# voichek/kmersGWAS

Hardware: AMD Instinct MI355X
Metric: k-mers x permutations scored/sec (higher is better)
Workload: dtype fp4 x fp6/fp4 block-scaled filter + f32/f64 exact re-score

## Files before the change

kmersgwas_amd/csrc/aux_kernels.hip:

```cpp
#include "score_common.h"
#include "synth.h"

namespace kgwas {

static hipError_t ensure_dyn_lds(const void* fn, size_t bytes) {
    if (bytes > 64 * 1024) return hipFuncSetAttribute(fn, hipFuncAttributeMaxDynamicSharedMemorySize, (int)bytes);
    return hipSuccess;
}

__global__ void __launch_bounds__(256) squeeze_kernel(const uint64_t* file_rows, uint64_t file_stride_w,
                                                      uint64_t n_rows, const uint32_t* colmap, uint32_t W_m,
                                                      uint32_t W_f, uint32_t* out) {
    extern __shared__ uint32_t lds_u32[];
    const uint32_t in_dw = 2u * W_f, in_ld = in_dw + 1u;
    const uint32_t out_dw = 2u * W_m, out_ld = out_dw + 1u;
    uint32_t* lin = lds_u32;
    uint32_t* lout = lds_u32 + 64u * in_ld;
    const uint64_t row0 = (uint64_t)blockIdx.x * 64u;
    const uint32_t* fr = reinterpret_cast<const uint32_t*>(file_rows);

    for (uint32_t e = threadIdx.x; e < 64u * in_dw; e += 256u) {
        const uint32_t rr = e / in_dw, dw = e - rr * in_dw;
        const uint64_t gr = row0 + rr;
        lin[rr * in_ld + dw] = (gr < n_rows) ? fr[gr * file_stride_w * 2u + 2u + dw] : 0u;
// ... 245 lines not shown
                                                         unsigned long long* __restrict__ h_tested, const double* __restrict__ thr, uint32_t n_thr,
                                                         double* __restrict__ h_thr) {
    for (uint32_t i = threadIdx.x; i < n_meta; i += 256u) h_meta[i] = meta[i];
    for (uint32_t i = threadIdx.x; i < n_tested; i += 256u) h_tested[i] = tested[i];
    for (uint32_t i = threadIdx.x; i < n_thr; i += 256u) h_thr[i] = thr[i];
}

hipError_t launch_chunk_tail(const uint32_t* meta, uint32_t n_meta, uint32_t* h_meta, const unsigned long long* tested, uint32_t n_tested,
                             unsigned long long* h_tested, const double* thr, uint32_t n_thr, double* h_thr, hipStream_t st) {
    launch_last(chunk_tail_kernel, dim3(1), dim3(256), 0, st, meta, n_meta, h_meta, tested, n_tested, h_tested, thr, n_thr, h_thr);
    return hipGetLastError();
}

__global__ void __launch_bounds__(256) thr_tail_kernel(const uint32_t* hist, const uint32_t* hist_base, uint32_t bins, const uint64_t* topn,
                                                       const double* thr_host, double* thr, const uint32_t* __restrict__ meta, uint32_t n_meta,
                                                       uint32_t* __restrict__ h_meta, const unsigned long long* __restrict__ tested, uint32_t n_tested,
                                                       unsigned long long* __restrict__ h_tested, double* __restrict__ h_thr) {
    thr_update_block(hist, hist_base, bins, topn, thr_host, thr, blockIdx.x);
    if (h_thr && threadIdx.x == 0) h_thr[blockIdx.x] = thr[blockIdx.x];
    if (blockIdx.x == 0) {
        for (uint32_t i = threadIdx.x; i < n_meta; i += 256u) h_meta[i] = meta[i];
        for (uint32_t i = threadIdx.x; i < n_tested; i += 256u) h_tested[i] = tested[i];
    }
}

hipError_t launch_thr_tail(const uint32_t* hist, const uint32_t* hist_base, uint32_t bins, const uint64_t* topn, const double* thr_host, double* thr,
                           uint32_t n_pheno, const uint32_t* meta, uint32_t n_meta, uint32_t* h_meta, const unsigned long long* tested,
                           uint32_t n_tested, unsigned long long* h_tested, double* h_thr, hipStream_t st) {
    if (n_pheno == 0 || bins % 256u) return hipErrorInvalidValue;
    launch_last(thr_tail_kernel, dim3(n_pheno), dim3(256), 0, st, hist, hist_base, bins, topn, thr_host, thr, meta, n_meta, h_meta, tested,
                n_tested, h_tested, h_thr);
    return hipGetLastError();
}

hipError_t launch_records_to_host(const double* sc, const uint64_t* km, const uint32_t* rw, uint32_t n, double* h_sc, uint64_t* h_km, uint32_t* h_rw,
                                  hipStream_t st) {
    if (!n) return hipSuccess;
    static const uint32_t max_blocks = (uint64_t)exp_int("KGWAS_RECORD_BLOCKS", 64u);
    const uint32_t blocks = std::min<uint32_t>((n + 255u) / 256u, std::max(1u, max_blocks));
    hipLaunchKernelGGL(records_to_host_kernel, dim3(blocks), dim3(256), 0, st, reinterpret_cast<const unsigned long long*>(sc),
                       reinterpret_cast<const unsigned long long*>(km), rw, n, reinterpret_cast<unsigned long long*>(h_sc),
                       reinterpret_cast<unsigned long long*>(h_km), h_rw);
    return hipGetLastError();
}

hipError_t launch_thr_update(const uint32_t* hist, const uint32_t* hist_base, uint32_t bins, const uint64_t* topn,
// ... 47 lines not shown
```

kmersgwas_amd/csrc/kernels.h:

```cpp
#pragma once
#include <hip/hip_runtime.h>
#include <stdint.h>

#include "env.h"
#include "launch.h"

namespace kgwas {

struct Cand {
    uint64_t kmer;
    double score;
    uint64_t row;
};

struct RowSrc {
    const uint32_t* base;
    uint64_t stride_dw;
    uint32_t off_dw;
    uint32_t avail_dw;
};

constexpr uint32_t TESTED_SHARDS = 256;

struct ScoreArgs {
// ... 20 lines not shown
    unsigned long long* tested;
    uint32_t* hist;
    const uint32_t* hist_base;
    uint32_t hist_bins;
    double* so_score;
    uint64_t* so_kmer;
    uint32_t* so_row;
};

constexpr int HIST_SHIFT = 44;
constexpr uint32_t HIST_BINS = 16384;

hipError_t launch_copy_to_host(const void* src, void* dst_dev, size_t bytes, hipStream_t st);
hipError_t launch_chunk_tail(const uint32_t* meta, uint32_t n_meta, uint32_t* h_meta, const unsigned long long* tested, uint32_t n_tested,
                             unsigned long long* h_tested, const double* thr, uint32_t n_thr, double* h_thr, hipStream_t st);
hipError_t launch_thr_tail(const uint32_t* hist, const uint32_t* hist_base, uint32_t bins, const uint64_t* topn, const double* thr_host, double* thr,
                           uint32_t n_pheno, const uint32_t* meta, uint32_t n_meta, uint32_t* h_meta, const unsigned long long* tested,
                           uint32_t n_tested, unsigned long long* h_tested, double* h_thr, hipStream_t st);
hipError_t launch_records_to_host(const double* sc, const uint64_t* km, const uint32_t* rw, uint32_t n, double* h_sc, uint64_t* h_km, uint32_t* h_rw,
                                  hipStream_t st);
hipError_t launch_thr_update(const uint32_t* hist, const uint32_t* hist_base, uint32_t bins, const uint64_t* topn,
                             const double* thr_host, double* thr, uint32_t n_pheno, hipStream_t st);

hipError_t launch_dense_select(const double* dense, const uint32_t* n1, uint32_t n_rows, uint32_t n_pheno, uint32_t S, uint32_t min_count,
                               const uint64_t* topn, double* thr_a, double* thr_b, double* thr_host_copy, uint32_t* info, hipStream_t st);

hipError_t launch_score_valu(const ScoreArgs& a, hipStream_t st);
hipError_t launch_score_mfma(const ScoreArgs& a, uint32_t rows_per_block, uint32_t nb_full, hipStream_t st);
size_t mfma_lds_bytes(uint32_t W_m);

struct CoarseCol {
    double kalpha;
    float iu;
// ... 73 lines not shown
    uint32_t S, n_pheno, min_count;
    uint32_t n_kgroups;
    const uint8_t* Bn;
    const NarrowCol* cols;
    const double* thr;
    unsigned long long* bitmap;
    uint64_t words_per_col;
    unsigned long long* tested;
    uint32_t row_off;
    uint32_t* seg_cnt;
    uint32_t n_segs;
    uint64_t slack_rows;
    uint32_t pack1;
};
hipError_t launch_bitmap_keys(unsigned long long* bitmap, uint64_t words_per_col, uint64_t n_rows, uint32_t n_pheno, uint32_t* blk_scratch,
                              unsigned long long* blk_mask, uint32_t* keys_sorted, uint32_t key_cap, uint32_t row_bits, uint32_t* surv_off,
                              uint32_t* surv_cnt, uint32_t* key_count, uint32_t* tile_pref, bool nibble_transposed, hipStream_t st);
hipError_t launch_narrow_keys(const unsigned long long* bitmap, uint64_t words_per_col, uint64_t n_rows, uint32_t n_pheno, const uint32_t* seg_cnt,
                              uint32_t* keys_sorted, uint32_t key_cap, uint32_t row_bits, uint32_t* surv_off, uint32_t* surv_cnt,
                              uint32_t* key_count, uint32_t* tile_pref, uint32_t* meta, const unsigned long long* tested_shards, hipStream_t st);
size_t narrow_lds_bytes(uint32_t n_kgroups);
hipError_t launch_narrow(const NarrowArgs& a, uint32_t rows_per_block, hipStream_t st);

hipError_t launch_pattern_hash(const RowSrc& src, const uint32_t* dmask, uint64_t n_rows, uint32_t S, uint32_t W_m,
                               uint32_t min_count, uint64_t* out, unsigned long long* out_count, hipStream_t st);
hipError_t count_distinct_u64(uint64_t* keys, uint64_t n, uint64_t* result, hipStream_t st);

hipError_t launch_bed_rowinfo(const uint32_t* sq, uint64_t n_rows, uint32_t W_m, uint32_t* n1_out, uint64_t* hash_out,
                              hipStream_t st);
hipError_t launch_bed_bytes(const uint32_t* sq, uint64_t n_rows, uint32_t W_m, uint32_t bytes_per_row, uint8_t* out,
                            hipStream_t st);

// ... 95 lines not shown
```

kmersgwas_amd/csrc/launch.h:

```cpp
#pragma once
#include <hip/hip_runtime.h>

#include <tuple>
#include <utility>

extern "C" hipError_t hipExtLaunchKernel(const void* function_address, dim3 numBlocks, dim3 dimBlocks, void** args, size_t sharedMemBytes,
                                         hipStream_t stream, hipEvent_t startEvent, hipEvent_t stopEvent, int flags);

namespace kgwas {

extern thread_local hipEvent_t g_bound_stop;

template <class... KA, size_t... I>
inline hipError_t launch_bound_impl(void (*kernel)(KA...), dim3 grid, dim3 block, size_t lds, hipStream_t st, hipEvent_t stop, std::tuple<KA...>& vals,
                                    std::index_sequence<I...>) {
    void* ptrs[] = {const_cast<void*>(static_cast<const void*>(&std::get<I>(vals)))..., nullptr};
    return hipExtLaunchKernel(reinterpret_cast<const void*>(kernel), grid, block, ptrs, lds, st, nullptr, stop, 0);
}

template <class... KA, class... A>
inline void launch_last(void (*kernel)(KA...), dim3 grid, dim3 block, size_t lds, hipStream_t st, A&&... args) {
    static_assert(sizeof...(KA) == sizeof...(A), "one argument per kernel parameter");
    const hipEvent_t stop = g_bound_stop;
    g_bound_stop = nullptr;
    if (!stop) {
        hipLaunchKernelGGL(kernel, grid, block, lds, st, static_cast<KA>(args)...);
        return;
    }
    std::tuple<KA...> vals(static_cast<KA>(args)...);
    (void)launch_bound_impl(kernel, grid, block, lds, st, stop, vals, std::index_sequence_for<KA...>{});
}

template <class F>
inline hipError_t bind_stop(hipEvent_t ev, hipStream_t st, F&& launcher) {
    g_bound_stop = ev;
    const hipError_t e = launcher();
    if (g_bound_stop) {
        g_bound_stop = nullptr;
        if (e == hipSuccess) return hipEventRecord(ev, st);
    }
    return e;
}

}
```

kmersgwas_amd/csrc/scan_create.cpp:

```cpp
#include "scan_internal.h"
#include <chrono>

struct CreateTrace {
    const bool on = opt_set("KGWAS_TRACE");
    const std::chrono::steady_clock::time_point t0 = std::chrono::steady_clock::now();
    void operator()(const char* what) const {
        if (on)
            fprintf(stderr, "[kgwas] scan_create +%.1f ms: %s\n", std::chrono::duration<double, std::milli>(std::chrono::steady_clock::now() - t0).count(), what);
    }
};

static std::unique_ptr<kgwas_scan> new_session(const kgwas_scan_params* p, ScanShape& sh) {
    if (p->struct_size != sizeof(kgwas_scan_params)) throw Error(KGWAS_ERR_ARG, "kgwas_scan_params: size mismatch");
    if (!p->col || !p->Y || !p->topn || p->n_acc == 0 || p->n_pheno == 0 || p->n_acc_file == 0)
        throw Error(KGWAS_ERR_ARG, "kgwas_scan_create: empty problem");
    if (p->n_acc > p->n_acc_file) throw Error(KGWAS_ERR_ARG, "more phenotyped accessions than table columns");
    if (p->n_acc_file >= (1ull << 31)) throw Error(KGWAS_ERR_ARG, "too many accessions");
    require_heap_emulation();
    check_device(p->device);
    KGWAS_HIP(hipSetDevice(p->device));
    std::unique_ptr<kgwas_scan> s(new kgwas_scan);
    s->device = p->device;
    s->S_f = p->n_acc_file;
    s->S = p->n_acc;
// ... 142 lines not shown
            if (pl.use_mx) s->st.coarse_mx = 1;
            s->st.coarse_mx_s1_fp6 = fs.s1_fp6;
            s->st.coarse_mx_steps = fs.n_steps;
        }
        M.ready = true;
    }
}

static void alloc_filter_buffers(kgwas_scan* s) {
    const uint64_t P = s->n_pheno;
    s->key_slots = (uint32_t)std::min<uint64_t>((uint64_t)s->cap * P, 0x7FFFFFFFull);
    s->d_surv_sorted.alloc(s->key_slots);
    s->bitmap_words = (s->chunk_max + 63) / 64;
    s->d_bitmap.alloc(P * s->bitmap_words);
    s->d_bm_blocks.alloc(P * ((s->bitmap_words + 1023) / 1024 + 1) + 4);
    if (!s->narrow) s->d_bm_mask.alloc(P * ((s->bitmap_words + 1023) / 1024) * 4 + 4);
    s->bitmap_clean = false;
    s->d_surv_cnt.alloc(P);
    s->d_surv_off.alloc(P);
    s->d_key_count.alloc(2);
    s->d_tile_pref.alloc(P + 1);
    s->d_tile_cnt.alloc((size_t)s->key_slots / 256 + P + 2);
    s->d_tmp_score.alloc(s->key_slots);
    int least = 0, greatest = 0;
    KGWAS_HIP(hipDeviceGetStreamPriorityRange(&least, &greatest));
    const bool hi = !(exp_int("KGWAS_COPY_PRIO", 1) == 0);
    KGWAS_HIP(hipStreamCreateWithPriority(&s->copy_stream, hipStreamNonBlocking, hi ? greatest : least));
    s->row_key_bits = 1;
    while (s->row_key_bits < 32 && (1ull << s->row_key_bits) < s->chunk_max) s->row_key_bits++;
}

// ... 172 lines not shown
```

kmersgwas_amd/csrc/scan_gpu.cpp:

```cpp
#include "scan_internal.h"

namespace kgwas {


void fill_args(kgwas_scan* s, ScoreArgs& a, const uint64_t* d_rows, uint64_t n_rows, uint64_t first_row,
               bool squeezed) {
    memset(&a, 0, sizeof(a));
    if (squeezed) {
        a.src.base = s->d_sq.p;
        a.src.stride_dw = 2 * s->W_m;
        a.src.off_dw = 0;
        a.src.avail_dw = (uint32_t)(2 * s->W_m);
    } else {
        a.src.base = reinterpret_cast<const uint32_t*>(d_rows);
        a.src.stride_dw = 2 * (1 + s->W_f);
        a.src.off_dw = 2;
        a.src.avail_dw = (uint32_t)(2 * s->W_f);
    }
    a.dmask = s->d_dmask.p;
    a.file_rows = d_rows;
    a.file_stride_w = 1 + s->W_f;
    a.n_rows = n_rows;
    a.first_row = first_row;
    a.S = (uint32_t)s->S;
// ... 302 lines not shown
            tu.hist = s->d_hist.p;
            tu.hist_base = s->d_hist_base.p;
            tu.bins = HIST_BINS;
            tu.topn = s->d_topn.p;
            tu.thr_host = s->d_thr_host.p;
            tu.thr = s->d_thr.p;
        }
        const bool zero_bitmap = use_coarse && (s->narrow || !s->bitmap_clean);
        const uint64_t zero_words = !zero_bitmap ? 0 : (s->narrow ? s->n_pheno * n_words : s->d_bitmap.n);
        const auto prep = [&] {
            return launch_chunk_prep(sl.d_cnt.p, (uint32_t)s->n_pheno, sl.d_tested.p, use_coarse ? s->d_key_count.p : nullptr,
                                     zero_bitmap ? s->d_bitmap.p : nullptr, zero_words,
                                     (use_coarse && s->narrow) ? s->d_bm_blocks.p : nullptr, (use_coarse && s->narrow) ? (uint32_t)s->n_pheno * n_segs : 0u,
                                     tu, s->stream);
        };
        if (s->direct) KGWAS_HIP(bind_stop(sl.ev_k0, s->stream, prep));
        else KGWAS_HIP(prep());
    }
    sl.used_coarse = use_coarse;
    if (use_coarse) {
        CoarseArgs c;
        memset(&c, 0, sizeof(c));
        c.src = a.src;
        c.n_rows = n_rows;
        c.S = a.S;
        c.n_pheno = a.n_pheno;
        c.min_count = a.min_count;
        c.n_kgroups = s->n_kgroups;
        const int cm = s->narrow ? 0 : pick_coarse_mode(s);
        if (s->dbg_keep_surv) dbg_log_thresholds(s, a.thr, n_rows, first_row, s->narrow ? 2u : (uint32_t)cm);
        const kgwas_scan::CoarseMode& M = s->cmode[cm];
        sl.coarse_mode = cm;
// ... 60 lines not shown
                    x.tested = c.tested;
                    x.eg_max = c.eg_max;
                    x.rall_max = c.rall_max;
                    x.rmax_max = c.rmax_max;
                    const auto filt = [&] {
                        return Pt.stream ? launch_mxs(x, Pt.T, Pt.ng, Pt.stream - 1u, rpb, s->stream) : launch_mx(x, Pt.T, rpb, s->stream);
                    };
                    if (last_part) KGWAS_HIP(bind_stop(sl.ev_mid, s->stream, filt));
                    else KGWAS_HIP(filt());
                } else {
                    const auto filt = [&] { return launch_coarse(c, Pt.T, rpb, s->stream); };
                    if (last_part) KGWAS_HIP(bind_stop(sl.ev_mid, s->stream, filt));
                    else KGWAS_HIP(filt());
                }
            }
            if (!M.n_parts) KGWAS_HIP(hipEventRecord(sl.ev_mid, s->stream));
        }
        a.tested = nullptr;
        a.so_score = sl.d_so_score.p;
        a.so_kmer = sl.d_so_kmer.p;
        a.so_row = sl.d_so_row.p;
        if (s->narrow) {
            KGWAS_HIP(launch_narrow_keys(s->d_bitmap.p, n_words, n_rows, (uint32_t)s->n_pheno, s->d_bm_blocks.p, s->d_surv_sorted.p, s->key_slots,
                                         s->row_key_bits, s->d_surv_off.p, s->d_surv_cnt.p, s->d_key_count.p, s->d_tile_pref.p, sl.d_meta.p, sl.d_tested.p, s->stream));
            if (s->dbg_keep_surv) dbg_log_survivors(s);
            KGWAS_HIP(bind_stop(sl.ev_k1, s->stream, [&] { return launch_rescore_direct(a, s->d_surv_sorted.p, s->d_surv_off.p, s->d_surv_cnt.p, s->row_key_bits, s->d_tile_pref.p, s->stream); }));
        } else {
        KGWAS_HIP(launch_bitmap_keys(s->d_bitmap.p, n_words, n_rows, (uint32_t)s->n_pheno, s->d_bm_blocks.p, s->d_bm_mask.p, s->d_surv_sorted.p, s->key_slots,
                                     s->row_key_bits, s->d_surv_off.p, s->d_surv_cnt.p, s->d_key_count.p, s->d_tile_pref.p, !s->narrow, s->stream));
        s->bitmap_clean = true;
        if (s->dbg_keep_surv) dbg_log_survivors(s);
        a.so_score = sl.d_so_score.p;
        a.so_kmer = sl.d_so_kmer.p;
        a.so_row = sl.d_so_row.p;
        KGWAS_HIP(bind_stop(sl.ev_k1, s->stream, [&] {
            return launch_rescore(a, s->d_surv_sorted.p, s->d_surv_off.p, s->d_surv_cnt.p, s->row_key_bits, s->d_tile_pref.p,
                                  s->d_tile_cnt.p, s->d_tmp_score.p, s->d_key_count.p, sl.d_meta.p, s->stream);
        }));
        }
        s->st.score_launches++;
    } else {
        if (s->direct) KGWAS_HIP(hipEventRecord(sl.ev_k0, s->stream));
        launch_score(s, a);
        KGWAS_HIP(hipEventRecord(sl.ev_k1, s->stream));
// ... 2 lines not shown
    static const bool tail_kernel = !(exp_int("KGWAS_TAIL_KERNEL", 1) == 0);
    const bool one_launch = use_coarse && tail_kernel && sl.h_meta_dev;
    const bool thr_and_tail = one_launch && s->hist_ready && !fused_tail;
    if (s->hist_ready && !fused_tail && !thr_and_tail)
        KGWAS_HIP(launch_thr_update(s->d_hist.p, s->d_hist_base.p, HIST_BINS, s->d_topn.p, s->d_thr_host.p, s->d_thr.p,
                                    (uint32_t)s->n_pheno, s->stream));
    if (!fused_tail && !one_launch)
        KGWAS_HIP(hipMemcpyAsync(sl.h_tested.p, sl.d_tested.p, TESTED_SHARDS * sizeof(unsigned long long), hipMemcpyDeviceToHost,
                                 s->stream));
    sl.tested_in_meta = fused_tail;
    if (thr_and_tail) {
        const bool thr_too = s->lazy_any.load(std::memory_order_relaxed);
        KGWAS_HIP(bind_stop(sl.ev_counts, s->stream, [&] {
            return launch_thr_tail(s->d_hist.p, s->d_hist_base.p, HIST_BINS, s->d_topn.p, s->d_thr_host.p, s->d_thr.p, (uint32_t)s->n_pheno, sl.d_meta.p,
                                   (uint32_t)(2 * s->n_pheno + 4), sl.h_meta_dev, sl.d_tested.p, (uint32_t)TESTED_SHARDS, sl.h_tested_dev,
                                   thr_too ? sl.h_thr_dev : nullptr, s->stream);
        }));
    } else if (one_launch) {
        const bool thr_too = s->lazy_any.load(std::memory_order_relaxed);
        KGWAS_HIP(bind_stop(sl.ev_counts, s->stream, [&] {
            return launch_chunk_tail(sl.d_meta.p, (uint32_t)(2 * s->n_pheno + 4), sl.h_meta_dev, sl.d_tested.p, fused_tail ? 0u : (uint32_t)TESTED_SHARDS,
                                     sl.h_tested_dev, s->d_thr.p, thr_too ? (uint32_t)s->n_pheno : 0u, sl.h_thr_dev, s->stream);
        }));
    } else if (use_coarse) {
        KGWAS_HIP(hipMemcpyAsync(sl.h_meta.p, sl.d_meta.p, (2 * s->n_pheno + 4) * sizeof(uint32_t), hipMemcpyDeviceToHost, s->stream));
        if (s->lazy_any.load(std::memory_order_relaxed))
            KGWAS_HIP(hipMemcpyAsync(sl.h_thr.p, s->d_thr.p, s->n_pheno * sizeof(double), hipMemcpyDeviceToHost, s->stream));
        KGWAS_HIP(hipEventRecord(sl.ev_counts, s->stream));
    } else {
        KGWAS_HIP(hipMemcpyAsync(sl.h_cnt.p, sl.d_cnt.p, s->n_pheno * sizeof(uint32_t), hipMemcpyDeviceToHost, s->stream));
        KGWAS_HIP(hipEventRecord(sl.ev_done, s->stream));
    }
// ... 19 lines not shown
        s->st.coarse_mode_rows[sl.coarse_mode] += sl.n_rows;
    }
    if (!s->direct) {
        float mq = 0;
        KGWAS_HIP(hipEventElapsedTime(&mq, sl.ev_sq0, sl.ev_k0));
        s->st.squeeze_kernel_ms += mq;
    }
    bool over = false;
    if (sl.used_coarse) {
        over = sl.h_meta.p[2 * s->n_pheno + 1] > s->key_slots;
    } else {
        for (uint64_t j = 0; j < s->n_pheno && !over; j++) over = sl.h_cnt.p[j] > s->cap;
    }
    if (s->trace) {
        uint64_t tot = 0, mx = 0;
        for (uint64_t q = 0; q < s->n_pheno; q++) {
            const uint64_t v = sl.used_coarse ? sl.h_meta.p[q] : sl.h_cnt.p[q];
            tot += v;
            mx = std::max<uint64_t>(mx, v);
        }
        fprintf(stderr, "[kgwas] chunk rows=%llu first=%llu kernel=%.3fms records %llu (max per column %llu)%s%s\n",
                (unsigned long long)sl.n_rows, (unsigned long long)sl.first_row, ms, (unsigned long long)tot,
                (unsigned long long)mx, sl.used_coarse ? (" survivors " + std::to_string(sl.h_meta.p[2 * s->n_pheno + 1])).c_str() : "",
                over ? " OVERFLOW" : "");
    }
    if (over) return false;
    if (sl.tested_in_meta)
        s->st.rows_tested += (uint64_t)sl.h_meta.p[2 * s->n_pheno + 2] | ((uint64_t)sl.h_meta.p[2 * s->n_pheno + 3] << 32);
    else
        for (uint32_t i = 0; i < TESTED_SHARDS; i++) s->st.rows_tested += sl.h_tested.p[i];
    return true;
}

uint64_t next_sparse_chunk(const kgwas_scan* s) {
    const double m = (double)std::max<uint64_t>(s->rows_submitted, 1);
    static const double fill_env = exp_num("KGWAS_FILL", 0.0);
    const double fill = fill_env > 0.0 ? fill_env : (s->narrow ? (s->lazy_any.load(std::memory_order_relaxed) ? 0.15 : 0.05) : 0.4);
// ... 98 lines not shown
```

kmersgwas_amd/csrc/scan_host.cpp:

```cpp
#include "scan_internal.h"
#include <sched.h>

namespace kgwas {

thread_local hipEvent_t g_bound_stop = nullptr;


std::vector<int> parse_cpulist(const char* path) {
    std::vector<int> out;
    FILE* f = fopen(path, "r");
    if (!f) return out;
    char buf[4096];
    if (fgets(buf, sizeof(buf), f)) {
        for (char* tok = strtok(buf, ",\n"); tok; tok = strtok(nullptr, ",\n")) {
            int a = 0, b = 0;
            const int k = sscanf(tok, "%d-%d", &a, &b);
            if (k == 1) b = a;
            if (k >= 1)
                for (int c = a; c <= b; c++) out.push_back(c);
        }
    }
    fclose(f);
    return out;
}
// ... 197 lines not shown
```

kmersgwas_amd/csrc/scan_internal.h:

```cpp
#pragma once
#include <algorithm>
#include <atomic>
#include <chrono>
#include <cmath>
#include <condition_variable>
#include <deque>
#include <limits>
#include <cstdio>
#include <cstdlib>
#include <cstring>
#include <functional>
#include <memory>
#include <mutex>
#include <string>
#include <thread>
#include <vector>

#include <dirent.h>
#include <immintrin.h>
#include <pthread.h>
#include <sched.h>
#include <sys/mman.h>

#include "common.h"
// ... 303 lines not shown
    double* so_score = nullptr;
    uint64_t* so_kmer = nullptr;
    uint32_t* so_row = nullptr;
    size_t ring_end = 0;
    DevBuf<double> d_so_score;
    DevBuf<uint64_t> d_so_kmer;
    DevBuf<uint32_t> d_so_row;
    DevBuf<uint32_t> d_meta;
    PinBuf<uint32_t> h_meta;
    uint32_t* h_meta_dev = nullptr;
    double* h_thr_dev = nullptr;
    unsigned long long* h_tested_dev = nullptr;
    PinBuf<double> h_thr;
    bool tie_check = false;
    bool tested_in_meta = false;
    hipEvent_t ev_counts = nullptr;
    DevBuf<unsigned long long> d_tested;
    PinBuf<unsigned long long> h_tested;
    hipEvent_t ev_sq0 = nullptr, ev_k0 = nullptr, ev_k1 = nullptr, ev_done = nullptr, ev_mid = nullptr;
    bool used_coarse = false;
    int coarse_mode = 0;
    double cand_est = 0;
    const uint64_t* rows = nullptr;
    uint64_t first_row = 0, n_rows = 0;
    bool squeezed = false, busy = false;
};

}

using namespace kgwas;
// ... 53 lines not shown
    PinBuf<uint32_t> h_sel_info;
    bool sel_valid = false;
    double infl_obs[2] = {4.0, 1.1};
    double mode_k = 0;
    std::chrono::steady_clock::time_point t_feed0;
    double t_ms() const { return std::chrono::duration<double, std::milli>(std::chrono::steady_clock::now() - t_feed0).count(); }
    uint64_t sum_topn = 0;
    bool narrow = false;
    bool narrow_pack1 = false;
    DevBuf<uint8_t> d_Bn;
    DevBuf<NarrowCol> d_ncols;
    DevBuf<unsigned long long> d_bitmap;
    uint64_t bitmap_words = 0;
    DevBuf<uint32_t> d_bm_blocks;
    DevBuf<unsigned long long> d_bm_mask;
    bool bitmap_clean = false;
    uint64_t slack_rows = 0;
    DevBuf<uint32_t> d_surv_sorted, d_surv_cnt, d_surv_off, d_key_count;
    DevBuf<uint32_t> d_tile_pref, d_tile_cnt;
    DevBuf<double> d_tmp_score;
    uint32_t key_slots = 0;
    uint32_t row_key_bits = 32;
    bool count_patterns = false;
    DevBuf<uint64_t> d_pat;
    DevBuf<unsigned long long> d_pat_cnt;
    uint64_t pat_upper = 0;
    Slot slot[MAX_SLOTS];
    PinBuf<uint8_t> ring;
    uint8_t* ring_dev = nullptr;
    bool streamed_feed = false;
// ... 208 lines not shown
```

kmersgwas_amd/csrc/score_narrow.hip:

```cpp
#include <stdlib.h>

#include <algorithm>

#include "score_common.h"

#ifndef KGWAS_NARROW_ABLATE
#define KGWAS_NARROW_ABLATE 0
#endif

namespace kgwas {

typedef int nv8i __attribute__((ext_vector_type(8)));
typedef float nv4f __attribute__((ext_vector_type(4)));

namespace {
constexpr int NRT = 4;
}

__device__ __forceinline__ void narrow_group(const uint32_t (&piece)[NRT][4], const uint4* sg, nv4f (&acc)[NRT]) {
#pragma unroll
    for (int j = 0; j < 4; j++) {
        uint4 s0, s1;
        if (KGWAS_NARROW_ABLATE & 16) {
            s0 = make_uint4(j, 1, 2, 3);
// ... 337 lines not shown
#undef NARROW_EACH
#undef NARROW_LOAD
#undef NARROW_PUT
    __syncthreads();
    narrow_flush_counts(a, L);
    if (a.tested) {
        uint32_t v = tested_local;
#pragma unroll
        for (int dd = 1; dd < 64; dd <<= 1) v += __shfl_xor(v, dd);
        if (lane == 0u && v) atomicAdd(&a.tested[blockIdx.x % TESTED_SHARDS], (unsigned long long)v);
    }
}

constexpr uint32_t BM_WORDS = 1024;

__global__ void __launch_bounds__(256) bitmap_count_kernel(const unsigned long long* bm, uint64_t words_per_col, uint32_t n_words,
                                                           uint32_t n_blocks, uint32_t* blk_cnt, unsigned long long* blk_mask) {
    __shared__ uint32_t part[4];
    const uint32_t p = blockIdx.y, b = blockIdx.x;
    const unsigned long long* w = bm + (uint64_t)p * words_per_col;
    uint32_t c = 0;
#pragma unroll
    for (int i = 0; i < 4; i++) {
        const uint32_t x = b * BM_WORDS + threadIdx.x * 4u + i;
        if (x < n_words) c += __popcll(w[x]);
    }
    const unsigned long long m = __ballot(c != 0u);
    if ((threadIdx.x & 63u) == 0u) blk_mask[((uint64_t)p * n_blocks + b) * 4u + (threadIdx.x >> 6)] = m;
#pragma unroll
    for (int d = 1; d < 64; d <<= 1) c += __shfl_xor(c, d);
    if ((threadIdx.x & 63u) == 0u) part[threadIdx.x >> 6] = c;
    __syncthreads();
    if (threadIdx.x == 0) blk_cnt[p * n_blocks + b] = part[0] + part[1] + part[2] + part[3];
}

__global__ void __launch_bounds__(256) bitmap_scan_kernel(uint32_t* blk_cnt, uint32_t n_blocks, uint32_t* col_total) {
    __shared__ uint32_t part[256];
    __shared__ uint32_t carry;
    const uint32_t p = blockIdx.x;
    if (threadIdx.x == 0) carry = 0;
    __syncthreads();
    for (uint32_t b0 = 0; b0 < n_blocks; b0 += 256u) {
        const uint32_t b = b0 + threadIdx.x;
        const uint32_t v = b < n_blocks ? blk_cnt[p * n_blocks + b] : 0u;
        part[threadIdx.x] = v;
        __syncthreads();
        for (uint32_t d = 1; d < 256u; d <<= 1) {
            const uint32_t x = threadIdx.x >= d ? part[threadIdx.x - d] : 0u;
            __syncthreads();
            part[threadIdx.x] += x;
            __syncthreads();
        }
        if (b < n_blocks) blk_cnt[p * n_blocks + b] = carry + part[threadIdx.x] - v;
        __syncthreads();
        if (threadIdx.x == 255u) carry += part[255];
        __syncthreads();
    }
    if (threadIdx.x == 0) col_total[p] = carry;
}

__device__ __forceinline__ void bitmap_bases_block(const uint32_t* col_total, uint32_t n_pheno, uint32_t key_cap, uint32_t* surv_off,
                                                   uint32_t* surv_cnt, uint32_t* key_count, uint32_t* tile_pref) {
    __shared__ uint32_t part[256];
    __shared__ uint32_t carry;
    if (threadIdx.x == 0) carry = 0;
    __syncthreads();
    for (uint32_t p0 = 0; p0 < n_pheno; p0 += 256u) {
        const uint32_t p = p0 + threadIdx.x;
        const uint32_t v = p < n_pheno ? col_total[p] : 0u;
        part[threadIdx.x] = v;
        __syncthreads();
        for (uint32_t d = 1; d < 256u; d <<= 1) {
            const uint32_t x = threadIdx.x >= d ? part[threadIdx.x - d] : 0u;
// ... 25 lines not shown
            const uint32_t x = threadIdx.x >= d ? part[threadIdx.x - d] : 0u;
            __syncthreads();
            part[threadIdx.x] += x;
            __syncthreads();
        }
        if (p < n_pheno) tile_pref[p] = carry + part[threadIdx.x] - v;
        __syncthreads();
        if (threadIdx.x == 255u) carry += part[255];
        __syncthreads();
    }
    if (threadIdx.x == 0) tile_pref[n_pheno] = carry;
    __syncthreads();
}

__global__ void __launch_bounds__(256) bitmap_scatter_kernel(unsigned long long* bm, uint64_t words_per_col, uint32_t n_words,
                                                             uint32_t n_blocks, const uint32_t* blk_off, const uint32_t* col_total,
                                                             const unsigned long long* blk_mask, uint32_t n_pheno, uint32_t* surv_off,
                                                             uint32_t* surv_cnt, uint32_t* key_count, uint32_t* tile_pref, uint32_t* keys,
                                                             uint32_t key_cap, uint32_t row_bits, bool nibble_transposed) {
    __shared__ uint32_t part[4];
    __shared__ uint32_t basep[4];
    const uint32_t p = blockIdx.y, b = blockIdx.x;
    if (p == 0u && b == 0u) bitmap_bases_block(col_total, n_pheno, key_cap, surv_off, surv_cnt, key_count, tile_pref);
    const uint32_t my_off = blk_off[p * n_blocks + b];
    const uint32_t next_off = b + 1u < n_blocks ? blk_off[p * n_blocks + b + 1u] : col_total[p];
    if (next_off == my_off) return;
    const uint32_t lane = threadIdx.x & 63u, wave = threadIdx.x >> 6;
    uint32_t col_base;
    {
        uint32_t v = 0;
        for (uint32_t q = threadIdx.x; q < p; q += 256u) v += col_total[q];
#pragma unroll
        for (int d = 1; d < 64; d <<= 1) v += __shfl_xor(v, d);
        if (lane == 0u) basep[wave] = v;
        __syncthreads();
        col_base = basep[0] + basep[1] + basep[2] + basep[3];
    }
    const bool mine = (blk_mask[((uint64_t)p * n_blocks + b) * 4u + wave] >> lane) & 1ull;
    unsigned long long* w = bm + (uint64_t)p * words_per_col;
    unsigned long long x[4] = {0ull, 0ull, 0ull, 0ull};
    uint32_t c = 0;
    if (mine) {
#pragma unroll
        for (int i = 0; i < 4; i++) {
            const uint32_t idx = b * BM_WORDS + threadIdx.x * 4u + i;
            if (idx < n_words) {
// ... 11 lines not shown
                for (int kg = 0; kg < 4; kg++)
#pragma unroll
                    for (int rt = 0; rt < 4; rt++) y |= ((x[i] >> (4 * (4 * kg + rt))) & 0xFull) << (4 * (4 * rt + kg));
                x[i] = y;
            }
        }
    }
    uint32_t incl = c;
#pragma unroll
    for (int d = 1; d < 64; d <<= 1) {
        const uint32_t t = __shfl_up(incl, d);
        if ((int)lane >= d) incl += t;
    }
    if (lane == 63u) part[wave] = incl;
    __syncthreads();
    uint32_t o = col_base + my_off + incl - c;
    for (uint32_t k = 0; k < wave; k++) o += part[k];
#pragma unroll
    for (int i = 0; i < 4; i++) {
        unsigned long long v = x[i];
        const uint32_t row0 = (b * BM_WORDS + threadIdx.x * 4u + i) * 64u;
        while (v) {
            const uint32_t bit = __ffsll((long long)v) - 1u;
            v &= v - 1ull;
            if (o < key_cap) keys[o] = (p << row_bits) | (row0 + bit);
            o++;
        }
    }
}

hipError_t launch_bitmap_keys(unsigned long long* bitmap, uint64_t words_per_col, uint64_t n_rows, uint32_t n_pheno, uint32_t* blk_scratch,
                              unsigned long long* blk_mask, uint32_t* keys_sorted, uint32_t key_cap, uint32_t row_bits, uint32_t* surv_off,
                              uint32_t* surv_cnt, uint32_t* key_count, uint32_t* tile_pref, bool nibble_transposed, hipStream_t st) {
    const uint32_t n_words = (uint32_t)((n_rows + 63) / 64);
    const uint32_t n_blocks = (n_words + BM_WORDS - 1) / BM_WORDS;
    hipLaunchKernelGGL(bitmap_count_kernel, dim3(n_blocks, n_pheno), dim3(256), 0, st, bitmap, words_per_col, n_words, n_blocks, blk_scratch, blk_mask);
    uint32_t* col_total = blk_scratch + (size_t)n_pheno * n_blocks;
    hipLaunchKernelGGL(bitmap_scan_kernel, dim3(n_pheno), dim3(256), 0, st, blk_scratch, n_blocks, col_total);
    hipLaunchKernelGGL(bitmap_scatter_kernel, dim3(n_blocks, n_pheno), dim3(256), 0, st, bitmap, words_per_col, n_words, n_blocks, blk_scratch,
                       col_total, blk_mask, n_pheno, surv_off, surv_cnt, key_count, tile_pref, keys_sorted, key_cap, row_bits, nibble_transposed);
    return hipGetLastError();
}

__global__ void __launch_bounds__(256) narrow_keys_kernel(const unsigned long long* bm, uint64_t words_per_col, uint32_t n_words, uint32_t n_segs,
                                                          uint32_t n_pheno, const uint32_t* seg_cnt, uint32_t* keys, uint32_t key_cap,
                                                          uint32_t row_bits, uint32_t* surv_off, uint32_t* surv_cnt, uint32_t* key_count,
                                                          uint32_t* tile_pref, uint32_t* meta, const unsigned long long* tested_shards) {
    __shared__ uint32_t red[4][NARROW_MAX_COLS + 1];
    __shared__ uint32_t tot[NARROW_MAX_COLS + 1];
    __shared__ uint32_t part[4];
    const uint32_t p = blockIdx.y, b = blockIdx.x;
    const uint32_t lane = threadIdx.x & 63u, wave = threadIdx.x >> 6;
    uint32_t cs[NARROW_MAX_COLS] = {0u, 0u, 0u, 0u}, mine = 0;
    for (uint32_t q = 0; q < n_pheno; q++)
        for (uint32_t k = threadIdx.x; k < n_segs; k += 256u) {
// ... 171 lines not shown
```

Baseline: 548.2 billion.

## Fold bitmap scan into count kernel and pre-zero counters in tail kernel

Removes the separate per-column bitmap scan kernel: the count kernel now handles eight blocks per workgroup and atomically accumulates column totals into a double-buffered totals array, and the scatter kernel computes its block prefix by summing earlier block counts directly. The previous chunk's tail kernel now also zeroes the tested shards, candidate counts and key counts, so the next chunk can skip its separate prep launch, with the timing event bound as a start event instead. This cuts kernel launches and serial work between stages, at the cost of an O(blocks) prefix sum in each scatter block and extra cross-chunk state that must stay consistent.

Measured after the change: 545.6 billion (median of 2 runs). Within noise of the previous version (-0.5%).

```diff
diff --git a/kmersgwas_amd/csrc/aux_kernels.hip b/kmersgwas_amd/csrc/aux_kernels.hip
--- a/kmersgwas_amd/csrc/aux_kernels.hip
+++ b/kmersgwas_amd/csrc/aux_kernels.hip
@@ -283,22 +283,30 @@
 
 __global__ void __launch_bounds__(256) thr_tail_kernel(const uint32_t* hist, const uint32_t* hist_base, uint32_t bins, const uint64_t* topn,
                                                        const double* thr_host, double* thr, const uint32_t* __restrict__ meta, uint32_t n_meta,
-                                                       uint32_t* __restrict__ h_meta, const unsigned long long* __restrict__ tested, uint32_t n_tested,
-                                                       unsigned long long* __restrict__ h_tested, double* __restrict__ h_thr) {
+                                                       uint32_t* __restrict__ h_meta, unsigned long long* tested, uint32_t n_tested,
+                                                       unsigned long long* __restrict__ h_tested, double* __restrict__ h_thr, TailPrep prep) {
     thr_update_block(hist, hist_base, bins, topn, thr_host, thr, blockIdx.x);
     if (h_thr && threadIdx.x == 0) h_thr[blockIdx.x] = thr[blockIdx.x];
     if (blockIdx.x == 0) {
         for (uint32_t i = threadIdx.x; i < n_meta; i += 256u) h_meta[i] = meta[i];
-        for (uint32_t i = threadIdx.x; i < n_tested; i += 256u) h_tested[i] = tested[i];
+        for (uint32_t i = threadIdx.x; i < n_tested; i += 256u) {
+            h_tested[i] = tested[i];
+            if (prep.cand_cnt) tested[i] = 0ull;
+        }
+        if (prep.cand_cnt) {
+            for (uint32_t i = threadIdx.x; i < prep.n_pheno; i += 256u) prep.cand_cnt[i] = 0u;
+            if (threadIdx.x < 2u && prep.key_count) prep.key_count[threadIdx.x] = 0u;
+        }
     }
 }
 
 hipError_t launch_thr_tail(const uint32_t* hist, const uint32_t* hist_base, uint32_t bins, const uint64_t* topn, const double* thr_host, double* thr,
-                           uint32_t n_pheno, const uint32_t* meta, uint32_t n_meta, uint32_t* h_meta, const unsigned long long* tested,
-                           uint32_t n_tested, unsigned long long* h_tested, double* h_thr, hipStream_t st) {
+                           uint32_t n_pheno, const uint32_t* meta, uint32_t n_meta, uint32_t* h_meta, unsigned long long* tested,
+                           uint32_t n_tested, unsigned long long* h_tested, double* h_thr, const TailPrep& prep, hipStream_t st) {
     if (n_pheno == 0 || bins % 256u) return hipErrorInvalidValue;
+    if (prep.cand_cnt && n_tested != TESTED_SHARDS) return hipErrorInvalidValue;
     launch_last(thr_tail_kernel, dim3(n_pheno), dim3(256), 0, st, hist, hist_base, bins, topn, thr_host, thr, meta, n_meta, h_meta, tested,
-                n_tested, h_tested, h_thr);
+                n_tested, h_tested, h_thr, prep);
     return hipGetLastError();
 }
 
diff --git a/kmersgwas_amd/csrc/kernels.h b/kmersgwas_amd/csrc/kernels.h
--- a/kmersgwas_amd/csrc/kernels.h
+++ b/kmersgwas_amd/csrc/kernels.h
@@ -58,9 +58,14 @@
 hipError_t launch_copy_to_host(const void* src, void* dst_dev, size_t bytes, hipStream_t st);
 hipError_t launch_chunk_tail(const uint32_t* meta, uint32_t n_meta, uint32_t* h_meta, const unsigned long long* tested, uint32_t n_tested,
                              unsigned long long* h_tested, const double* thr, uint32_t n_thr, double* h_thr, hipStream_t st);
+struct TailPrep {
+    uint32_t* cand_cnt;
+    uint32_t n_pheno;
+    uint32_t* key_count;
+};
 hipError_t launch_thr_tail(const uint32_t* hist, const uint32_t* hist_base, uint32_t bins, const uint64_t* topn, const double* thr_host, double* thr,
-                           uint32_t n_pheno, const uint32_t* meta, uint32_t n_meta, uint32_t* h_meta, const unsigned long long* tested,
-                           uint32_t n_tested, unsigned long long* h_tested, double* h_thr, hipStream_t st);
+                           uint32_t n_pheno, const uint32_t* meta, uint32_t n_meta, uint32_t* h_meta, unsigned long long* tested,
+                           uint32_t n_tested, unsigned long long* h_tested, double* h_thr, const TailPrep& prep, hipStream_t st);
 hipError_t launch_records_to_host(const double* sc, const uint64_t* km, const uint32_t* rw, uint32_t n, double* h_sc, uint64_t* h_km, uint32_t* h_rw,
                                   hipStream_t st);
 hipError_t launch_thr_update(const uint32_t* hist, const uint32_t* hist_base, uint32_t bins, const uint64_t* topn,
@@ -164,8 +169,8 @@
     uint32_t pack1;
 };
 hipError_t launch_bitmap_keys(unsigned long long* bitmap, uint64_t words_per_col, uint64_t n_rows, uint32_t n_pheno, uint32_t* blk_scratch,
-                              unsigned long long* blk_mask, uint32_t* keys_sorted, uint32_t key_cap, uint32_t row_bits, uint32_t* surv_off,
-                              uint32_t* surv_cnt, uint32_t* key_count, uint32_t* tile_pref, bool nibble_transposed, hipStream_t st);
+                              unsigned long long* blk_mask, uint32_t* col_total, uint32_t* next_total, uint32_t* keys_sorted, uint32_t key_cap, uint32_t row_bits, uint32_t* surv_off, uint32_t* surv_cnt,
+                              uint32_t* key_count, uint32_t* tile_pref, bool nibble_transposed, hipStream_t st);
 hipError_t launch_narrow_keys(const unsigned long long* bitmap, uint64_t words_per_col, uint64_t n_rows, uint32_t n_pheno, const uint32_t* seg_cnt,
                               uint32_t* keys_sorted, uint32_t key_cap, uint32_t row_bits, uint32_t* surv_off, uint32_t* surv_cnt,
                               uint32_t* key_count, uint32_t* tile_pref, uint32_t* meta, const unsigned long long* tested_shards, hipStream_t st);
diff --git a/kmersgwas_amd/csrc/launch.h b/kmersgwas_amd/csrc/launch.h
--- a/kmersgwas_amd/csrc/launch.h
+++ b/kmersgwas_amd/csrc/launch.h
@@ -10,25 +10,27 @@
 namespace kgwas {
 
 extern thread_local hipEvent_t g_bound_stop;
+extern thread_local hipEvent_t g_bound_start;
 
 template <class... KA, size_t... I>
 inline hipError_t launch_bound_impl(void (*kernel)(KA...), dim3 grid, dim3 block, size_t lds, hipStream_t st, hipEvent_t stop, std::tuple<KA...>& vals,
-                                    std::index_sequence<I...>) {
+                                    hipEvent_t start, std::index_sequence<I...>) {
     void* ptrs[] = {const_cast<void*>(static_cast<const void*>(&std::get<I>(vals)))..., nullptr};
-    return hipExtLaunchKernel(reinterpret_cast<const void*>(kernel), grid, block, ptrs, lds, st, nullptr, stop, 0);
+    return hipExtLaunchKernel(reinterpret_cast<const void*>(kernel), grid, block, ptrs, lds, st, start, stop, 0);
 }
 
 template <class... KA, class... A>
 inline void launch_last(void (*kernel)(KA...), dim3 grid, dim3 block, size_t lds, hipStream_t st, A&&... args) {
     static_assert(sizeof...(KA) == sizeof...(A), "one argument per kernel parameter");
-    const hipEvent_t stop = g_bound_stop;
+    const hipEvent_t stop = g_bound_stop, start = g_bound_start;
     g_bound_stop = nullptr;
-    if (!stop) {
+    g_bound_start = nullptr;
+    if (!stop && !start) {
         hipLaunchKernelGGL(kernel, grid, block, lds, st, static_cast<KA>(args)...);
         return;
     }
     std::tuple<KA...> vals(static_cast<KA>(args)...);
-    (void)launch_bound_impl(kernel, grid, block, lds, st, stop, vals, std::index_sequence_for<KA...>{});
+    (void)launch_bound_impl(kernel, grid, block, lds, st, stop, vals, start, std::index_sequence_for<KA...>{});
 }
 
 template <class F>
@@ -42,4 +44,11 @@
     return e;
 }
 
+inline void bind_start(hipEvent_t ev) { g_bound_start = ev; }
+inline bool bound_start_taken() {
+    const bool taken = g_bound_start == nullptr;
+    g_bound_start = nullptr;
+    return taken;
 }
+
+}
diff --git a/kmersgwas_amd/csrc/scan_create.cpp b/kmersgwas_amd/csrc/scan_create.cpp
--- a/kmersgwas_amd/csrc/scan_create.cpp
+++ b/kmersgwas_amd/csrc/scan_create.cpp
@@ -180,7 +180,12 @@
     s->bitmap_words = (s->chunk_max + 63) / 64;
     s->d_bitmap.alloc(P * s->bitmap_words);
     s->d_bm_blocks.alloc(P * ((s->bitmap_words + 1023) / 1024 + 1) + 4);
-    if (!s->narrow) s->d_bm_mask.alloc(P * ((s->bitmap_words + 1023) / 1024) * 4 + 4);
+    if (!s->narrow) {
+        s->d_bm_mask.alloc(P * ((s->bitmap_words + 1023) / 1024) * 4 + 4);
+        s->d_bm_totals.alloc(2 * P);
+        KGWAS_HIP(hipMemset(s->d_bm_totals.p, 0, s->d_bm_totals.n * sizeof(uint32_t)));
+        KGWAS_HIP(hipStreamSynchronize(nullptr));
+    }
     s->bitmap_clean = false;
     s->d_surv_cnt.alloc(P);
     s->d_surv_off.alloc(P);
diff --git a/kmersgwas_amd/csrc/scan_gpu.cpp b/kmersgwas_amd/csrc/scan_gpu.cpp
--- a/kmersgwas_amd/csrc/scan_gpu.cpp
+++ b/kmersgwas_amd/csrc/scan_gpu.cpp
@@ -340,8 +340,17 @@
                                      (use_coarse && s->narrow) ? s->d_bm_blocks.p : nullptr, (use_coarse && s->narrow) ? (uint32_t)s->n_pheno * n_segs : 0u,
                                      tu, s->stream);
         };
-        if (s->direct) KGWAS_HIP(bind_stop(sl.ev_k0, s->stream, prep));
-        else KGWAS_HIP(prep());
+        const bool prepared = use_coarse && !s->narrow && sl.prepared && !zero_bitmap;
+        sl.prepared = false;
+        if (prepared) {
+            if (s->direct) bind_start(sl.ev_k0);
+        } else if (s->direct) {
+            KGWAS_HIP(bind_stop(sl.ev_k0, s->stream, prep));
+        } else {
+            KGWAS_HIP(prep());
+        }
+        if (zero_bitmap && !s->narrow)
+            KGWAS_HIP(hipMemsetAsync(s->d_bm_totals.p, 0, s->d_bm_totals.n * sizeof(uint32_t), s->stream));
     }
     sl.used_coarse = use_coarse;
     if (use_coarse) {
@@ -432,6 +441,7 @@
                     else KGWAS_HIP(filt());
                 }
             }
+            if (!bound_start_taken()) KGWAS_HIP(hipEventRecord(sl.ev_k0, s->stream));
             if (!M.n_parts) KGWAS_HIP(hipEventRecord(sl.ev_mid, s->stream));
         }
         a.tested = nullptr;
@@ -444,8 +454,9 @@
             if (s->dbg_keep_surv) dbg_log_survivors(s);
             KGWAS_HIP(bind_stop(sl.ev_k1, s->stream, [&] { return launch_rescore_direct(a, s->d_surv_sorted.p, s->d_surv_off.p, s->d_surv_cnt.p, s->row_key_bits, s->d_tile_pref.p, s->stream); }));
         } else {
-        KGWAS_HIP(launch_bitmap_keys(s->d_bitmap.p, n_words, n_rows, (uint32_t)s->n_pheno, s->d_bm_blocks.p, s->d_bm_mask.p, s->d_surv_sorted.p, s->key_slots,
-                                     s->row_key_bits, s->d_surv_off.p, s->d_surv_cnt.p, s->d_key_count.p, s->d_tile_pref.p, !s->narrow, s->stream));
+        KGWAS_HIP(launch_bitmap_keys(s->d_bitmap.p, n_words, n_rows, (uint32_t)s->n_pheno, s->d_bm_blocks.p, s->d_bm_mask.p, s->d_bm_totals.p + (s->bm_flip & 1u) * s->n_pheno,
+                                     s->d_bm_totals.p + ((s->bm_flip + 1u) & 1u) * s->n_pheno, s->d_surv_sorted.p, s->key_slots, s->row_key_bits, s->d_surv_off.p, s->d_surv_cnt.p, s->d_key_count.p, s->d_tile_pref.p, !s->narrow, s->stream));
+        s->bm_flip++;
         s->bitmap_clean = true;
         if (s->dbg_keep_surv) dbg_log_survivors(s);
         a.so_score = sl.d_so_score.p;
@@ -478,8 +489,9 @@
         KGWAS_HIP(bind_stop(sl.ev_counts, s->stream, [&] {
             return launch_thr_tail(s->d_hist.p, s->d_hist_base.p, HIST_BINS, s->d_topn.p, s->d_thr_host.p, s->d_thr.p, (uint32_t)s->n_pheno, sl.d_meta.p,
                                    (uint32_t)(2 * s->n_pheno + 4), sl.h_meta_dev, sl.d_tested.p, (uint32_t)TESTED_SHARDS, sl.h_tested_dev,
-                                   thr_too ? sl.h_thr_dev : nullptr, s->stream);
+                                   thr_too ? sl.h_thr_dev : nullptr, TailPrep{sl.d_cnt.p, (uint32_t)s->n_pheno, s->d_key_count.p}, s->stream);
         }));
+        sl.prepared = true;
     } else if (one_launch) {
         const bool thr_too = s->lazy_any.load(std::memory_order_relaxed);
         KGWAS_HIP(bind_stop(sl.ev_counts, s->stream, [&] {
@@ -529,13 +541,15 @@
     }
     if (s->trace) {
         uint64_t tot = 0, mx = 0;
+        float mf = 0;
+        if (sl.used_coarse) KGWAS_HIP(hipEventElapsedTime(&mf, sl.ev_k0, sl.ev_mid));
         for (uint64_t q = 0; q < s->n_pheno; q++) {
             const uint64_t v = sl.used_coarse ? sl.h_meta.p[q] : sl.h_cnt.p[q];
             tot += v;
             mx = std::max<uint64_t>(mx, v);
         }
-        fprintf(stderr, "[kgwas] chunk rows=%llu first=%llu kernel=%.3fms records %llu (max per column %llu)%s%s\n",
-                (unsigned long long)sl.n_rows, (unsigned long long)sl.first_row, ms, (unsigned long long)tot,
+        fprintf(stderr, "[kgwas] chunk rows=%llu first=%llu kernel=%.3fms filter=%.3fms records %llu (max per column %llu)%s%s\n",
+                (unsigned long long)sl.n_rows, (unsigned long long)sl.first_row, ms, mf, (unsigned long long)tot,
                 (unsigned long long)mx, sl.used_coarse ? (" survivors " + std::to_string(sl.h_meta.p[2 * s->n_pheno + 1])).c_str() : "",
                 over ? " OVERFLOW" : "");
     }
diff --git a/kmersgwas_amd/csrc/scan_host.cpp b/kmersgwas_amd/csrc/scan_host.cpp
--- a/kmersgwas_amd/csrc/scan_host.cpp
+++ b/kmersgwas_amd/csrc/scan_host.cpp
@@ -4,6 +4,7 @@
 namespace kgwas {
 
 thread_local hipEvent_t g_bound_stop = nullptr;
+thread_local hipEvent_t g_bound_start = nullptr;
 
 
 std::vector<int> parse_cpulist(const char* path) {
diff --git a/kmersgwas_amd/csrc/scan_internal.h b/kmersgwas_amd/csrc/scan_internal.h
--- a/kmersgwas_amd/csrc/scan_internal.h
+++ b/kmersgwas_amd/csrc/scan_internal.h
@@ -341,6 +341,7 @@
     PinBuf<double> h_thr;
     bool tie_check = false;
     bool tested_in_meta = false;
+    bool prepared = false;
     hipEvent_t ev_counts = nullptr;
     DevBuf<unsigned long long> d_tested;
     PinBuf<unsigned long long> h_tested;
@@ -424,6 +425,8 @@
     uint64_t bitmap_words = 0;
     DevBuf<uint32_t> d_bm_blocks;
     DevBuf<unsigned long long> d_bm_mask;
+    DevBuf<uint32_t> d_bm_totals;
+    uint32_t bm_flip = 0;
     bool bitmap_clean = false;
     uint64_t slack_rows = 0;
     DevBuf<uint32_t> d_surv_sorted, d_surv_cnt, d_surv_off, d_key_count;
diff --git a/kmersgwas_amd/csrc/score_narrow.hip b/kmersgwas_amd/csrc/score_narrow.hip
--- a/kmersgwas_amd/csrc/score_narrow.hip
+++ b/kmersgwas_amd/csrc/score_narrow.hip
@@ -375,49 +375,42 @@
 
 constexpr uint32_t BM_WORDS = 1024;
 
+constexpr uint32_t BM_GROUP = 8;
 __global__ void __launch_bounds__(256) bitmap_count_kernel(const unsigned long long* bm, uint64_t words_per_col, uint32_t n_words,
-                                                           uint32_t n_blocks, uint32_t* blk_cnt, unsigned long long* blk_mask) {
-    __shared__ uint32_t part[4];
-    const uint32_t p = blockIdx.y, b = blockIdx.x;
+                                                           uint32_t n_blocks, uint32_t* blk_cnt, unsigned long long* blk_mask,
+                                                           uint32_t* col_total) {
+    __shared__ uint32_t part[BM_GROUP][4];
+    const uint32_t p = blockIdx.y, b0 = blockIdx.x * BM_GROUP;
+    const uint32_t lane = threadIdx.x & 63u, wave = threadIdx.x >> 6;
     const unsigned long long* w = bm + (uint64_t)p * words_per_col;
+    unsigned long long v[BM_GROUP][4];
+#pragma unroll
+    for (uint32_t i = 0; i < BM_GROUP; i++)
+#pragma unroll
+        for (uint32_t j = 0; j < 4; j++) {
+            const uint32_t x = (b0 + i) * BM_WORDS + threadIdx.x * 4u + j;
+            v[i][j] = x < n_words ? w[x] : 0ull;
+        }
+#pragma unroll
+    for (uint32_t i = 0; i < BM_GROUP; i++) {
+        uint32_t c = __popcll(v[i][0]) + __popcll(v[i][1]) + __popcll(v[i][2]) + __popcll(v[i][3]);
+        const unsigned long long m = __ballot(c != 0u);
+        if (lane == 0u && b0 + i < n_blocks) blk_mask[((uint64_t)p * n_blocks + b0 + i) * 4u + wave] = m;
+#pragma unroll
+        for (int d = 1; d < 64; d <<= 1) c += __shfl_xor(c, d);
+        if (lane == 0u) part[i][wave] = c;
+    }
+    __syncthreads();
     uint32_t c = 0;
-#pragma unroll
-    for (int i = 0; i < 4; i++) {
-        const uint32_t x = b * BM_WORDS + threadIdx.x * 4u + i;
-        if (x < n_words) c += __popcll(w[x]);
-    }
-    const unsigned long long m = __ballot(c != 0u);
-    if ((threadIdx.x & 63u) == 0u) blk_mask[((uint64_t)p * n_blocks + b) * 4u + (threadIdx.x >> 6)] = m;
-#pragma unroll
-    for (int d = 1; d < 64; d <<= 1) c += __shfl_xor(c, d);
-    if ((threadIdx.x & 63u) == 0u) part[threadIdx.x >> 6] = c;
-    __syncthreads();
-    if (threadIdx.x == 0) blk_cnt[p * n_blocks + b] = part[0] + part[1] + part[2] + part[3];
-}
-
-__global__ void __launch_bounds__(256) bitmap_scan_kernel(uint32_t* blk_cnt, uint32_t n_blocks, uint32_t* col_total) {
-    __shared__ uint32_t part[256];
-    __shared__ uint32_t carry;
-    const uint32_t p = blockIdx.x;
-    if (threadIdx.x == 0) carry = 0;
-    __syncthreads();
-    for (uint32_t b0 = 0; b0 < n_blocks; b0 += 256u) {
-        const uint32_t b = b0 + threadIdx.x;
-        const uint32_t v = b < n_blocks ? blk_cnt[p * n_blocks + b] : 0u;
-        part[threadIdx.x] = v;
-        __syncthreads();
-        for (uint32_t d = 1; d < 256u; d <<= 1) {
-            const uint32_t x = threadIdx.x >= d ? part[threadIdx.x - d] : 0u;
-            __syncthreads();
-            part[threadIdx.x] += x;
-            __syncthreads();
-        }
-        if (b < n_blocks) blk_cnt[p * n_blocks + b] = carry + part[threadIdx.x] - v;
-        __syncthreads();
-        if (threadIdx.x == 255u) carry += part[255];
-        __syncthreads();
-    }
-    if (threadIdx.x == 0) col_total[p] = carry;
+    if (threadIdx.x < BM_GROUP && b0 + threadIdx.x < n_blocks) {
+        c = part[threadIdx.x][0] + part[threadIdx.x][1] + part[threadIdx.x][2] + part[threadIdx.x][3];
+        blk_cnt[p * n_blocks + b0 + threadIdx.x] = c;
+    }
+    if (wave == 0u) {
+#pragma unroll
+        for (int d = 1; d < (int)BM_GROUP; d <<= 1) c += __shfl_xor(c, d);
+        if (lane == 0u && c) atomicAdd(&col_total[p], c);
+    }
 }
 
 __device__ __forceinline__ void bitmap_bases_block(const uint32_t* col_total, uint32_t n_pheno, uint32_t key_cap, uint32_t* surv_off,
@@ -473,22 +466,24 @@
 }
 
 __global__ void __launch_bounds__(256) bitmap_scatter_kernel(unsigned long long* bm, uint64_t words_per_col, uint32_t n_words,
-                                                             uint32_t n_blocks, const uint32_t* blk_off, const uint32_t* col_total,
-                                                             const unsigned long long* blk_mask, uint32_t n_pheno, uint32_t* surv_off,
+                                                             uint32_t n_blocks, const uint32_t* blk_cnt, const uint32_t* col_total,
+                                                             uint32_t* next_total, const unsigned long long* blk_mask, uint32_t n_pheno, uint32_t* surv_off,
                                                              uint32_t* surv_cnt, uint32_t* key_count, uint32_t* tile_pref, uint32_t* keys,
                                                              uint32_t key_cap, uint32_t row_bits, bool nibble_transposed) {
     __shared__ uint32_t part[4];
     __shared__ uint32_t basep[4];
     const uint32_t p = blockIdx.y, b = blockIdx.x;
-    if (p == 0u && b == 0u) bitmap_bases_block(col_total, n_pheno, key_cap, surv_off, surv_cnt, key_count, tile_pref);
-    const uint32_t my_off = blk_off[p * n_blocks + b];
-    const uint32_t next_off = b + 1u < n_blocks ? blk_off[p * n_blocks + b + 1u] : col_total[p];
-    if (next_off == my_off) return;
+    if (p == 0u && b == 0u) {
+        bitmap_bases_block(col_total, n_pheno, key_cap, surv_off, surv_cnt, key_count, tile_pref);
+        for (uint32_t q = threadIdx.x; q < n_pheno; q += 256u) next_total[q] = 0u;
+    }
+    if (blk_cnt[p * n_blocks + b] == 0u) return;
     const uint32_t lane = threadIdx.x & 63u, wave = threadIdx.x >> 6;
     uint32_t col_base;
     {
         uint32_t v = 0;
         for (uint32_t q = threadIdx.x; q < p; q += 256u) v += col_total[q];
+        for (uint32_t q = threadIdx.x; q < b; q += 256u) v += blk_cnt[p * n_blocks + q];
 #pragma unroll
         for (int d = 1; d < 64; d <<= 1) v += __shfl_xor(v, d);
         if (lane == 0u) basep[wave] = v;
@@ -530,7 +525,7 @@
     }
     if (lane == 63u) part[wave] = incl;
     __syncthreads();
-    uint32_t o = col_base + my_off + incl - c;
+    uint32_t o = col_base + incl - c;
     for (uint32_t k = 0; k < wave; k++) o += part[k];
 #pragma unroll
     for (int i = 0; i < 4; i++) {
@@ -546,15 +541,15 @@
 }
 
 hipError_t launch_bitmap_keys(unsigned long long* bitmap, uint64_t words_per_col, uint64_t n_rows, uint32_t n_pheno, uint32_t* blk_scratch,
-                              unsigned long long* blk_mask, uint32_t* keys_sorted, uint32_t key_cap, uint32_t row_bits, uint32_t* surv_off,
-                              uint32_t* surv_cnt, uint32_t* key_count, uint32_t* tile_pref, bool nibble_transposed, hipStream_t st) {
+                              unsigned long long* blk_mask, uint32_t* col_total, uint32_t* next_total, uint32_t* keys_sorted, uint32_t key_cap, uint32_t row_bits, uint32_t* surv_off, uint32_t* surv_cnt,
+                              uint32_t* key_count, uint32_t* tile_pref, bool nibble_transposed, hipStream_t st) {
     const uint32_t n_words = (uint32_t)((n_rows + 63) / 64);
     const uint32_t n_blocks = (n_words + BM_WORDS - 1) / BM_WORDS;
-    hipLaunchKernelGGL(bitmap_count_kernel, dim3(n_blocks, n_pheno), dim3(256), 0, st, bitmap, words_per_col, n_words, n_blocks, blk_scratch, blk_mask);
-    uint32_t* col_total = blk_scratch + (size_t)n_pheno * n_blocks;
-    hipLaunchKernelGGL(bitmap_scan_kernel, dim3(n_pheno), dim3(256), 0, st, blk_scratch, n_blocks, col_total);
+    hipLaunchKernelGGL(bitmap_count_kernel, dim3((n_blocks + BM_GROUP - 1) / BM_GROUP, n_pheno), dim3(256), 0, st, bitmap, words_per_col, n_words,
+                       n_blocks, blk_scratch, blk_mask, col_total);
     hipLaunchKernelGGL(bitmap_scatter_kernel, dim3(n_blocks, n_pheno), dim3(256), 0, st, bitmap, words_per_col, n_words, n_blocks, blk_scratch,
-                       col_total, blk_mask, n_pheno, surv_off, surv_cnt, key_count, tile_pref, keys_sorted, key_cap, row_bits, nibble_transposed);
+                       col_total, next_total, blk_mask, n_pheno, surv_off, surv_cnt, key_count, tile_pref, keys_sorted, key_cap, row_bits,
+                       nibble_transposed);
     return hipGetLastError();
 }
 
```
